# AI4Science-WestlakeU/RealPDEBench

Measured on AMD Instinct MI355X. Metric: train-step samples/sec (+ autoregressive rollout fields/sec in 'rollout'), FNO cylinder 128^2, higher is better.
Workload: dtype f32 storage / split-bf16x3 MFMA contractions (six bf16 products per fp32 product, fp32 accumulate), fp32-grade

## Files before the change

### include/rpb.h

```cpp
#ifndef RPB_H
#define RPB_H
#ifdef __cplusplus
extern "C" {
#endif

#define RPB_OK 0
#define RPB_ERR_ARG (-1)
#define RPB_ERR_LAUNCH (-2)
#define RPB_ERR_UNSUPPORTED (-3)

#define RPB_ABI_VERSION 3
const char* rpb_last_error(void);
int rpb_abi_version(void);
int rpb_bf16_const_planes(void);

int rpb_lift_pad_fwd(const float* x, const float* gt, const float* gh, const float* gw, const float* fc0_w,
                     const float* fc0_b, float* out, int B, int T, int H, int W, int Cin, int C, int Tp, int Hp, int Wp,
                     void* stream);
int rpb_lift_bwd_rows(void);
int rpb_lift_bwd(const float* g_out, const float* x, const float* gt, const float* gh, const float* gw, float* part,
                 int B, int T, int H, int W, int Cin, int C, int Tp, int Hp, int Wp, void* stream);

int rpb_axis_gemm(const float* in, float* out, const float* Mt, int G, int K, int O, int N, long in_g_stride,
                  long in_k_stride, long out_g_stride, long out_o_stride, int k_valid, int accumulate,
// ... 167 lines not shown
int rpb_col_reduce(const float* x, int ldx, float* part, int F, long n, int C, int mode, void* stream);

int rpb_feat_mix(const float* Phi, const float* w0, const float* b0, float* Xh, int B, int M2, int NB, int Cin, int C, void* stream);
int rpb_feat_mix_wgrad_rows(void);
int rpb_feat_mix_wgrad(const float* G, const float* Phi, float* part, int B, int M2, int NB, int Cin, int C, void* stream);
int rpb_small_gemm(const float* A, const float* Bm, float* out, int M, int N, int K, int a_rs, int a_cs, int b_rs, int b_cs,
                   int ldo, int accumulate, void* stream);
int rpb_lift_feat(const float* x, const float* gt, const float* gh, const float* gw, float* out, int B, int T, int H, int W,
                  int Cin, int Tp, int Hp, int Wp, int FW, void* stream);
int rpb_cell_mix_feat(const float* phi, const float* Wcomp, const float* bias, const float* z2, const float* GWt, float* out,
                      float* stats_part, long ncell, int FW, int K2, int Wp, const float* oxf_mean, const float* oxf_invstd,
                      const float* oxf_gamma, const float* oxf_beta, int oxf_gelu, void* stream);
int rpb_bn_bwd_row_feat(const float* s, const float* gy, const float* phi, float* gs, const float* mean, const float* invstd,
                        const float* gamma, const float* beta, const float* sums, double count, int gelu, const float* GWt,
                        float* Y1, float* part, int G, int Wp, int C, int K2, int FW, void* stream);

int rpb_bn_bwd_row_c128_supported(int Wp, int K2);
int rpb_bn_bwd_row_c128(const float* s, const float* gy, float* gs, const float* mean, const float* invstd, const float* gamma,
                        const float* beta, const float* sums, double count, int gelu, const float* GWt, float* Y1, float* part,
                        int G, int Wp, int K2, void* stream);

int rpb_proj_bwd_fused_supported(int C, int DO, int W, int Wp);
long rpb_proj_dgrad_slots(int B, int Tp, int Hp);
int rpb_proj_dgrad(const float* s, const float* w1, const float* gu, float* g, float* stats_part, int B, int DO, int T, int H, int W,
                   int Tp, int Hp, int Wp, const float* xf_mean, const float* xf_invstd, const float* xf_gamma, const float* xf_beta,
                   int xf_gelu, void* stream);

int rpb_head_bwd_supported(int C, int DO, int W, int Wp, int xf_gelu, int act);
long rpb_head_bwd_slots(int B, int T, int H);
int rpb_head_bwd_row(int DO);
// ... 140 lines not shown
```

### realpdebench_amd/_lib.py

```python
import ctypes
import os

_HERE = os.path.dirname(os.path.abspath(__file__))
ABI_VERSION = 3
LIB_PATH = os.environ.get("RPB_LIB_PATH") or os.path.join(_HERE, "csrc", "librpb_hip.so")

_P, _I, _L, _F, _D = ctypes.c_void_p, ctypes.c_int, ctypes.c_long, ctypes.c_float, ctypes.c_double
_T = {"p": _P, "i": _I, "l": _L, "f": _F, "d": _D}

SIGNATURES = {
    "rpb_last_error": (ctypes.c_char_p, ""),
    "rpb_abi_version": (_I, ""),
    "rpb_bf16_const_planes": (_I, ""),
    "rpb_lift_pad_fwd": (_I, "ppppppp" + "iiiiiiiii" + "p"),
    "rpb_lift_pad_fwd_bf16": (_I, "ppppppp" + "iiiiiiiii" + "p"),
    "rpb_axis_gemm_bf16in": (_I, "ppp" + "iiii" + "llll" + "i" + "p"),
    "rpb_cell_mix_bf16": (_I, "pppppp" + "l" + "iii" + "ppppi" + "i" + "p"),
    "rpb_axis_gemm_bf16out": (_I, "ppp" + "iiii" + "llll" + "i" + "p"),
    "rpb_proj_fwd_bf16": (_I, "pppppp" + "l" + "ii" + "iiiiii" + "i" + "p"),
    "rpb_spectrum_bin": (_I, "ppiip"),
    "rpb_feat_mix": (_I, "pppp" + "iiiii" + "p"),
    "rpb_feat_mix_wgrad_rows": (_I, ""),
    "rpb_feat_mix_wgrad": (_I, "ppp" + "iiiii" + "p"),
    "rpb_small_gemm": (_I, "ppp" + "iiiiiiiii" + "p"),
    "rpb_lift_feat": (_I, "ppppp" + "iiiiiiiii" + "p"),
    "rpb_cell_mix_feat": (_I, "ppppppp" + "l" + "iii" + "ppppi" + "p"),
    "rpb_bn_bwd_row_feat": (_I, "ppppppppp" + "d" + "i" + "ppp" + "iiiii" + "p"),
    "rpb_proj_bwd_fused_supported": (_I, "iiii"),
    "rpb_proj_dgrad_slots": (_L, "iii"),
    "rpb_proj_dgrad": (_I, "ppppp" + "ii" + "iiiiii" + "ppppi" + "p"),
    "rpb_stream_probe": (_I, "pppp" + "l" + "ii" + "p"),
    "rpb_mfma_probe": (_I, "pp" + "ii" + "p" + "p"),
    "rpb_head_bwd_supported": (_I, "iiiiii"),
    "rpb_head_bwd_slots": (_L, "iii"),
    "rpb_head_bwd_row": (_I, "i"),
    "rpb_head_bwd": (_I, "ppppppp" + "ii" + "iiiiii" + "pppp" + "p"),
    "rpb_head_bwd_finalize": (_I, "pppp" + "i" + "ppppp" + "p"),
    "rpb_head_fwd_bwd": (_I, "pppppp" + "f" + "ppp" + "ii" + "iiiiii" + "pppp" + "p"),
# ... 225 lines not shown
```

### realpdebench_amd/csrc/rpb_bwd_row.hip

```cpp
#include "rpb_common.h"
#include "rpb_bwr.h"
#include <stdlib.h>

template <int N>
struct RowVec;
template <>
struct RowVec<1> {
    typedef float T;
    typedef unsigned U;
};
template <>
struct RowVec<2> {
    typedef f32x2 T;
    typedef unsigned U __attribute__((ext_vector_type(2)));
};

template <int NT>
__device__ __forceinline__ typename RowVec<NT>::T row_load(rsrc_t r, int voff, int soff) {
    if constexpr (NT == 1) return __builtin_bit_cast(float, __builtin_amdgcn_raw_buffer_load_b32(r, voff, soff, RPB_STREAM_AUX));
    else return __builtin_bit_cast(f32x2, __builtin_amdgcn_raw_buffer_load_b64(r, voff, soff, RPB_STREAM_AUX));
}
template <int NT>
__device__ __forceinline__ void row_store(typename RowVec<NT>::T v, rsrc_t r, int voff, int soff) {
    if constexpr (NT == 1) __builtin_amdgcn_raw_buffer_store_b32(__builtin_bit_cast(unsigned, v), r, voff, soff, RPB_STREAM_AUX);
// ... 18 lines not shown
    const float* mean;
    const float* invstd;
    const float* gamma;
    const float* beta;
    const float* sums;
    float inv_count;
    int gelu;
    XForm xf;
    const float* GWt;
    float* Y1;
    float* part;
    int G, Wp, K2;
    int feat_w;
};

template <int C, bool FEAT = false>
__global__ __launch_bounds__(512) void bwd_row_kernel(BwdRowArgs a) {
    constexpr int NT = C / 32;
    typedef typename RowVec<NT>::T vec;
    extern __shared__ float Ml[];
    const int Wp = a.Wp, K2 = a.K2;
    const int nchunk = (Wp + 7) / 8;
    const int Kp = nchunk * 8;
    for (int idx = threadIdx.x; idx < Kp * 32; idx += blockDim.x) {
        const int k = idx >> 5, o = idx & 31;
        Ml[idx] = (k < Wp && o < K2) ? a.GWt[k * K2 + o] : 0.f;
    }
    __syncthreads();

    const int waves = blockDim.x >> 6;
    const int wave = __builtin_amdgcn_readfirstlane(threadIdx.x >> 6);
    const int lane = threadIdx.x & 63;
    const int col = lane & 31, half = lane >> 5;
    const long slot = (long)blockIdx.x * waves + wave;
    const long nslots = (long)gridDim.x * waves;
    const bool gelu = a.gelu != 0;
    const bool has_xf = !FEAT && a.xf.mean != nullptr;
    const int FW = a.feat_w;

    float mu[NT], is[NT], ga[NT], be[NT], m1[NT], m2[NT];
    XParam xp[NT];
#pragma unroll
    for (int t = 0; t < NT; ++t) {
        const int ch = col * NT + t;
        mu[t] = a.mean[ch];
        is[t] = a.invstd[ch];
        ga[t] = a.gamma[ch];
        be[t] = a.beta[ch];
        m1[t] = a.sums[ch] * a.inv_count;
        m2[t] = a.sums[C + ch] * a.inv_count;
        if (has_xf) xp[t] = xf_load(a.xf, ch);
    }
    f32x16 dW[NT][NT];
    float bsum[NT];
#pragma unroll
    for (int o = 0; o < NT; ++o) {
        bsum[o] = 0.f;
#pragma unroll
        for (int i = 0; i < NT; ++i) dW[o][i] = zero16();
    }

    const int voff = (half * C + col * NT) * 4;
    const unsigned row_bytes = (unsigned)Wp * C * 4;
    vec sa[4], ya[4], xa[4], sb[4], yb[4], xb[4];

    for (long g_ = slot; g_ < a.G; g_ += nslots) {
        const long g = (long)__builtin_amdgcn_readfirstlane((int)g_);
        const long off = g * (long)Wp * C;
        const rsrc_t rs = make_rsrc(a.s + off, row_bytes);
        const rsrc_t ry = make_rsrc(a.gy + off, row_bytes);
        const rsrc_t rx = FEAT ? make_rsrc(a.x + g * (long)Wp * FW, (unsigned)Wp * FW * 4u) : make_rsrc(a.x + off, row_bytes);
        const rsrc_t ro = make_rsrc(a.gs ? a.gs + off : a.s, a.gs ? row_bytes : 0u);
        f32x16 accw[NT];
#pragma unroll
        for (int t = 0; t < NT; ++t) accw[t] = zero16();

        auto load_chunk = [&](int c, vec (&sv)[4], vec (&yv)[4], vec (&xv)[4]) {
            const int vo = voff + c * 8 * C * 4;
#pragma unroll
            for (int j = 0; j < 4; ++j) {
                sv[j] = row_load<NT>(rs, vo + 2 * j * C * 4, 0);
                yv[j] = row_load<NT>(ry, vo + 2 * j * C * 4, 0);
                if (FEAT) {
                    const int fo = col < FW ? ((c * 8 + 2 * j + half) * FW + col) * 4 : 0x7ffffff0;
                    rset<NT>(xv[j], 0, buf_load_f32(rx, fo, 0));
                } else {
                    xv[j] = row_load<NT>(rx, vo + 2 * j * C * 4, 0);
                }
            }
        };
        auto compute_chunk = [&](int c, const vec (&sv)[4], const vec (&yv)[4], const vec (&xv)[4]) {
            const int vo = voff + c * 8 * C * 4;
            const float* mp = Ml + (c * 8 + half) * 32 + col;
#pragma unroll
            for (int j = 0; j < 4; ++j) {
                const bool valid = c * 8 + 2 * j + half < Wp;
                float gsv[NT], xt[NT];
                vec gout;
                if constexpr (NT == 2) {
                    const f32x2 isv = f32x2{is[0], is[1]}, gav = f32x2{ga[0], ga[1]};
                    const f32x2 sh = (sv[j] - f32x2{mu[0], mu[1]}) * isv;
                    f32x2 gz = yv[j];
                    if (gelu) gz = gz * gelu_grad2(pk_fma(sh, gav, f32x2{be[0], be[1]}));
                    f32x2 v = (gav * isv) * ((gz - f32x2{m1[0], m1[1]}) - sh * f32x2{m2[0], m2[1]});
                    v = valid ? v : pk2(0.f);
                    gout = v;
                    gsv[0] = v[0];
                    gsv[1] = v[1];
                    if (FEAT) {
                        xt[0] = xv[j][0];
                        xt[1] = 0.f;
                    } else {
                        f32x2 xx = xv[j];
                        if (has_xf) {
// ... 5 lines not shown
                        xt[1] = xx[1];
                    }
                } else {
#pragma unroll
                for (int t = 0; t < NT; ++t) {
                    const float sh = (rget<NT>(sv[j], t) - mu[t]) * is[t];
                    const float gyv = rget<NT>(yv[j], t);
                    const float gz = gelu ? gyv * gelu_grad_f(sh * ga[t] + be[t]) : gyv;
                    const float v = ga[t] * is[t] * (gz - m1[t] - sh * m2[t]);
                    gsv[t] = valid ? v : 0.f;
                    rset<NT>(gout, t, gsv[t]);
                    const float xv0 = (FEAT && t > 0) ? 0.f : rget<NT>(xv[j], t);
                    xt[t] = has_xf ? xf_apply(xv0, xp[t], a.xf.gelu != 0) : xv0;
                }
                }
                row_store<NT>(gout, ro, vo + 2 * j * C * 4, 0);
                const float aw = mp[2 * j * 32];
#pragma unroll
                for (int t = 0; t < NT; ++t) accw[t] = mfma32(aw, gsv[t], accw[t]);
#pragma unroll
                for (int o = 0; o < NT; ++o) {
                    bsum[o] += gsv[o];
#pragma unroll
                    for (int i = 0; i < (FEAT ? 1 : NT); ++i) dW[o][i] = mfma32(gsv[o], xt[i], dW[o][i]);
                }
            }
        };
        load_chunk(0, sa, ya, xa);
        for (int c = 0; c < nchunk; c += 2) {
            if (c + 1 < nchunk) load_chunk(c + 1, sb, yb, xb);
            compute_chunk(c, sa, ya, xa);
            if (c + 2 < nchunk) load_chunk(c + 2, sa, ya, xa);
            if (c + 1 < nchunk) compute_chunk(c + 1, sb, yb, xb);
        }
        float* yp = a.Y1 + g * (long)K2 * C + col * NT;
#pragma unroll
        for (int r = 0; r < 16; ++r) {
            const int o = mfma_row(lane, r);
            if (o < K2) {
                vec v;
#pragma unroll
                for (int t = 0; t < NT; ++t) rset<NT>(v, t, accw[t][r]);
                *reinterpret_cast<vec*>(yp + (long)o * C) = v;
            }
        }
    }
    float* part = a.part + slot * ((long)C * C + C);
#pragma unroll
    for (int o = 0; o < NT; ++o) {
#pragma unroll
        for (int i = 0; i < (FEAT ? 1 : NT); ++i)
#pragma unroll
            for (int r = 0; r < 16; ++r)
                part[(long)(mfma_row(lane, r) * NT + o) * C + (FEAT ? col : col * NT + i)] = dW[o][i][r];
        const float b = bsum[o] + __shfl_xor(bsum[o], 32, 64);
        if (half == 0) part[(long)C * C + col * NT + o] = b;
    }
}

extern "C" long rpb_bn_bwd_row_slots(int G) {
    const long slots = (long)rpb_num_cus() * 8;
    const long need = ((long)G + 7) / 8 * 8;
    return slots < need ? slots : need;
}

extern "C" int rpb_bn_bwd_row(const float* s, const float* gy, const float* x, float* gs, const float* mean,
                              const float* invstd, const float* gamma, const float* beta, const float* sums,
                              double count, int gelu, const float* xf_mean, const float* xf_invstd,
                              const float* xf_gamma, const float* xf_beta, int xf_gelu, const float* GWt, float* Y1,
                              float* part, int G, int Wp, int C, int K2, void* stream) {
    RPB_REQUIRE(s && gy && gs && mean && invstd && gamma && beta && sums && GWt && Y1 && part,
// ... 35 lines not shown
        BwrArgs b;
        b.s = s; b.gy = gy; b.x = nullptr; b.gs = gs;
        b.mean = mean + 64 * h; b.invstd = invstd + 64 * h; b.gamma = gamma + 64 * h; b.beta = beta + 64 * h; b.sums = sums + 64 * h;
        b.inv_count = (float)(1.0 / count); b.gelu = gelu; b.xf = XForm{nullptr, nullptr, nullptr, nullptr, 0};
        b.GW = GWt; b.Y1 = Y1; b.part = part + h * rows * (64 * 64 + 64); b.G = G; b.Wp = Wp; b.K2 = K2; b.CS = 128; b.coff = 64 * h;
        const int rc = rpb_bwr_launch(b, rows, (hipStream_t)stream);
        if (rc != RPB_OK) return rc;
    }
    return RPB_OK;
}

extern "C" int rpb_bn_bwd_row_feat(const float* s, const float* gy, const float* phi, float* gs, const float* mean,
                                   const float* invstd, const float* gamma, const float* beta, const float* sums, double count,
                                   int gelu, const float* GWt, float* Y1, float* part, int G, int Wp, int C, int K2, int FW,
                                   void* stream) {
    RPB_REQUIRE(s && gy && phi && mean && invstd && gamma && beta && sums && GWt && Y1 && part, "bn_bwd_row_feat: null pointer");
    RPB_REQUIRE(C == 64 && (FW == 8 || FW == 32), "bn_bwd_row_feat: C=%d FW=%d unsupported", C, FW);
    RPB_REQUIRE(G > 0 && Wp > 0 && K2 > 0 && K2 <= 32 && count > 0, "bn_bwd_row_feat: bad sizes G=%d Wp=%d K2=%d", G, Wp, K2);
    BwdRowArgs a;
    a.s = s; a.gy = gy; a.x = phi; a.gs = gs; a.mean = mean; a.invstd = invstd; a.gamma = gamma; a.beta = beta;
    a.sums = sums; a.inv_count = (float)(1.0 / count); a.gelu = gelu;
    a.xf = XForm{nullptr, nullptr, nullptr, nullptr, 0};
    a.GWt = GWt; a.Y1 = Y1; a.part = part; a.G = G; a.Wp = Wp; a.K2 = K2; a.feat_w = FW;
    const int grid = (int)(rpb_bn_bwd_row_slots(G) / 8);
    const size_t lds = (size_t)((Wp + 7) / 8 * 8) * 32 * 4;
    hipLaunchKernelGGL((bwd_row_kernel<64, true>), dim3(grid), dim3(512), lds, (hipStream_t)stream, a);
    RPB_CHECK_LAUNCH("bn_bwd_row_feat");
}
```

### realpdebench_amd/dft.py

```python
import math

import numpy as np
import torch


def kept_modes(n, m, two_sided):
    ks = list(range(m))
    if two_sided:
        if 2 * m > n:
            raise ValueError(f"modes {m} overlap on an axis of length {n} (2*modes must be <= padded size)")
        ks += list(range(n - m, n))
    elif m > n // 2 + 1:
        raise ValueError(f"modes {m} exceed the rfft length {n // 2 + 1}")
    return ks


def _fwd_complex(n, ks):
    k = np.asarray(ks, dtype=np.float64)[:, None]
    p = np.arange(n, dtype=np.float64)[None, :]
    th = 2.0 * math.pi * ((k * p) % n) / n
    c, s = np.cos(th), np.sin(th)
    M = np.zeros((2, len(ks), n, 2))
    M[0, :, :, 0] = c
    M[0, :, :, 1] = s
# ... 41 lines not shown
        self.kw = kept_modes(Wp, m3, False)
        self.KT, self.KH, self.KW = len(self.kt), len(self.kh), len(self.kw)
        self.M = self.KT * self.KH * self.KW
        mats = {
            "FW": _fwd_real(Wp, self.kw),
            "FH": _fwd_complex(Hp, self.kh),
            "FT": _fwd_complex(Tp, self.kt),
            "GT": _inv_complex(Tp, self.kt),
            "GH": _inv_complex(Hp, self.kh),
            "GW": _inv_real(Wp, self.kw, float(Tp) * Hp * Wp),
        }
        for name, m in mats.items():
            t = torch.from_numpy(np.ascontiguousarray(m)).to(torch.float32)
            setattr(self, name, t.to(device).contiguous())
            setattr(self, name + "t", t.t().contiguous().to(device))


def ref_weights_to_mode_major(w1, w2, w3, w4):
    top = torch.cat([w1, w3], dim=3)
    bot = torch.cat([w2, w4], dim=3)
    full = torch.cat([top, bot], dim=2)
    full = full.permute(2, 3, 4, 0, 1).contiguous()
    return torch.view_as_real(full).reshape(-1, full.shape[3], full.shape[4], 2).contiguous()


def mode_major_to_ref_weights(wm, modes):
    m1, m2, m3 = modes
    Ci, Co = wm.shape[1], wm.shape[2]
    full = torch.view_as_complex(wm.reshape(2 * m1, 2 * m2, m3, Ci, Co, 2).contiguous())
    full = full.permute(3, 4, 0, 1, 2)
# ... 6 lines not shown
```

### realpdebench_amd/model/fno.py

```python
import math
import os
from collections import OrderedDict

import numpy as np
import torch
import torch.nn as nn

from .. import ops
from ..dft import SpectralPlan, mode_major_to_ref_weights, ref_weights_to_mode_major
from .model import Model

HID = 128
BN_EPS = 1e-5
BN_MOMENTUM = 0.1
_ALIGN = 64


class _Workspace:

    def __init__(self, model, B, training, device):
        d = ops.Dims(B, *model.shape_in[:3], model.dim_in, model.width, model.padding)
        self.d, self.training = d, training
        self.bf16 = (not training) and model.storage == "bf16"
        self.arith = model.arith if (not training and not self.bf16) else "f32"
# ... 44 lines not shown
            phi[..., c0 + 1] = grids[1].view(1, H_, 1)
            phi[..., c0 + 2] = grids[2].view(1, 1, W_)
            phi[..., c0 + 3] = 1.0
            self.phi = phi
            n1 = 2 * plan.KW * self.NB
            self.fy1 = torch.empty(T_ * H_ * n1, **f)
            self.fy2 = torch.empty(T_ * 2 * plan.KH * plan.KW * self.NB, **f)
            self.PhiH = torch.empty(2 * plan.M * self.NB, **f)
            if training:
                self.fm_rows = ops.feat_mix_wgrad_rows()
                self.fm_part = torch.empty(self.fm_rows * C * (Cin + 4), **f)
                self.fm_sum = torch.empty(C * (Cin + 4), **f)
                self.mgf = torch.empty(C * (Cin + 3) + C, **f)
                self.mgf2 = torch.empty(C * C, **f)
                self.dconv = torch.empty(C * (Cin + 4), **f)
        if training:
            self.G = [torch.empty(d.ncell, C, **f) for _ in range(2)]
            self.proj_gu = (C == 64 and type(model)._lift_fwd is FNO3d._lift_fwd
                            and ops.proj_bwd_fused_supported(C, model.dim_out, d.W, d.Wp))
            self.head_fused = (C == 64 and type(model)._lift_fwd is FNO3d._lift_fwd and
                               ops.head_bwd_supported(C, model.dim_out, d.W, d.Wp, False, model.proj_act))
            self.gu = None if self.head_fused else torch.empty(d.ncrop, HID, **f)
            if self.proj_gu:
                self.pd_slots = ops.proj_dgrad_slots(d)
            if self.head_fused:
                self.hb_slots, self.hb_row = ops.head_bwd_slots(d), ops.head_bwd_row(model.dim_out)
                self.hb_part = torch.empty(self.hb_slots * self.hb_row, **f)
                self.hb_tot = torch.empty(self.hb_row, **f)
                self.hb_loss_part = torch.empty(self.hb_slots, **f)
                self.head_loss_fused = model.dim_out <= 2
# ... 310 lines not shown
        world = self.dp.world_size if (self.dp is not None and training) else 1
        a_in, xf = ws.A0, None
        y1_ready = False
        for l in range(L):
            s = ws.S[l] if training else ws.S[l % 2]
            xh = ws.Xh[l] if training else ws.Xh[0]
            if dpw is not None:
                dpw.params_ready(dpw.layer_bucket(l))
            if l == 0 and ws.feat0:
                self._feature_spectrum(x, ws, plan)
                ops.feat_mix(ws.PhiH, P("fc0.weight"), P("fc0.bias"), xh, d.B, 2 * plan.M, ws.NB, self.dim_in, C)
            elif y1_ready:
                self._spectral_forward_stages(a_in, ws, xh, (None, plan.FHt, plan.FTt), first_layer=False, y1=ws.Y1f)
            else:
                self._spectral_forward_stages(a_in, ws, xh, (plan.FWt, plan.FHt, plan.FTt), first_layer=(l == 0), xf=xf)
            ops.mode_contract_fwd(xh, P(f"spec.{l}"), ws.Yh, d.B, plan.M, C)
            self._spectral_inverse_stages(ws.Yh, ws, (plan.GTt, plan.GHt))
            if training:
                if l == 0 and ws.featfull:
                    ops.cell_mix_feat(ws.phic, ws.wcomp, P("convs.0.bias"), ws.Y1, plan.GWt, s, ws.stat_part, d.ncell, ws.FW,
                                      2 * plan.KW, d.Wp)
                else:
                    ops.cell_mix(a_in, P(f"convs.{l}.weight"), P(f"convs.{l}.bias"), ws.Y1, plan.GWt, s, ws.stat_part,
                                 d.ncell, C, C, 2 * plan.KW, d.Wp, xf=xf)
                ops.reduce_partials(ws.stat_part, ws.stat_rows, 2 * C, out_f64=ws.sums64)
                if world > 1 or (self.dp is not None and training and getattr(self.dp, "sync_stats_always", False)):
                    self.dp.all_reduce_sum(ws.sums64)
                ops.bn_finalize(ws.sums64, float(d.ncell) * world, BN_EPS, BN_MOMENTUM, ws.mean[l], ws.invstd[l],
                                self.bn_running_mean[l], self.bn_running_var[l], C)
                self.bn_num_batches_tracked[l] += 1
                a_in, xf = s, self._layer_xf(ws, l, True)
            else:
                ops.bn_eval_prep(self.bn_running_var[l], BN_EPS, ws.invstd[l], C)
                y1_ready = False
                if ws.fuse_w and l < L - 1 and (l > 0 or ws.featfull or ws.bf16):
                    feat = l == 0 and ws.featfull
                    ops.cell_mix_eval_dft(ws.phic if feat else a_in, ws.wcomp if feat else P(f"convs.{l}.weight"), P(f"convs.{l}.bias"),
                                          ws.Z2, plan.GWt, s, d.ncell, 2 * plan.KW, d.Wp, self._layer_xf(ws, l, False), plan.FWt,
                                          2 * plan.KW, ws.Y1f, feat_w=ws.FW if feat else 0, arith=ws.arith, spec_e=ops.spec_exp(d))
                    y1_ready = True
                elif l == 0 and ws.featfull:
                    ops.cell_mix_feat(ws.phic, ws.wcomp, P("convs.0.bias"), ws.Z2, plan.GWt, s, None, d.ncell, ws.FW,
                                      2 * plan.KW, d.Wp, oxf=self._layer_xf(ws, l, False))
# ... 62 lines not shown
                ops.cell_mix(ws.gu, P("fc1.weight"), None, None, None, g, ws.bn_part, d.ncell, HID, C, 0, 1, transpose_w=True,
                             gather=True, crop6=d.crop6, bnb=(ws.S[L - 1],) + self._layer_xf(ws, L - 1, True))
                ops.reduce_partials(ws.bn_part, ws.bnb_rows_gather, 2 * C, out_f32=ws.bn_sums)
        gz_ok = ws.fused_bwd and ops.cell_mix_writes_gz(d.ncell, C, C, 2 * plan.KW, d.Wp, True)
        g_is_gz = False
        for l in range(L - 1, -1, -1):
            gelu = l < L - 1 and not g_is_gz
            gam, bet = P(f"bns.{l}.weight"), P(f"bns.{l}.bias")
            GP(f"bns.{l}.bias").copy_(ws.bn_sums[:C])
            GP(f"bns.{l}.weight").copy_(ws.bn_sums[C:])
            if world > 1 or (self.dp is not None and getattr(self.dp, "sync_stats_always", False)):
                self.dp.all_reduce_sum(ws.bn_sums)
            a_in = ws.A0 if l == 0 else ws.S[l - 1]
            xf_in = None if l == 0 else self._layer_xf(ws, l - 1, True)
            feat_l0 = l == 0 and ws.featfull
            if feat_l0:
                ops.bn_bwd_row_feat(ws.S[l], g, ws.phic, None if ws.feat0 else g, ws.mean[l], ws.invstd[l], gam, bet, ws.bn_sums,
                                    float(d.ncell) * world, gelu, plan.GW, ws.Y1, ws.wg_part, d.B * d.Tp * d.Hp, d.Wp, C,
                                    2 * plan.KW, ws.FW)
            elif ws.fused_bwd:
                wg_later = ws.wg_in_cmx and l > 0
                ops.bn_bwd_row(ws.S[l], g, None if wg_later else a_in, g, ws.mean[l], ws.invstd[l], gam, bet, ws.bn_sums,
                               float(d.ncell) * world, gelu, xf_in, plan.GW, ws.Y1, ws.wg_part, d.B * d.Tp * d.Hp,
                               d.Wp, C, 2 * plan.KW)
            elif ws.row128:
                ops.bn_bwd_row_c128(ws.S[l], g, g, ws.mean[l], ws.invstd[l], gam, bet, ws.bn_sums, float(d.ncell) * world, gelu,
                                    plan.GW, ws.Y1, ws.row128_part, d.B * d.Tp * d.Hp, d.Wp, 2 * plan.KW)
                ops.cell_wgrad(g, a_in, ws.wg_part, d.ncell, C, C, xf=xf_in)
            else:
                ops.bn_bwd_apply(ws.S[l], g, ws.mean[l], ws.invstd[l], gam, bet, ws.bn_sums, float(d.ncell) * world,
                                 g, d.ncell, C, gelu)
                ops.cell_wgrad(g, a_in, ws.wg_part, d.ncell, C, C, xf=xf_in)
            partc = ws.wg_part[:ws.wg_rows_c * (C * C + C)].view(ws.wg_rows_c, C * C + C)
            if feat_l0:
                self._reduce_cols(partc, 0, C * C, ws.mgf2)
                ops.small_gemm(ws.mgf2, ws.w0ext, GP("convs.0.weight"), C, C, ws.FW, C, 1, 1, ws.FW, C)
            elif not (ws.fused_bwd and ws.wg_in_cmx and l > 0):
                self._reduce_cols(partc, 0, C * C, GP(f"convs.{l}.weight"))
            self._reduce_cols(partc, C * C, C, GP(f"convs.{l}.bias"))
            self._spectral_forward_stages(g, ws, ws.Yh, (None if (ws.fused_bwd or ws.row128) else plan.GW, plan.GH, plan.GT),
                                          first_layer=False)
            ops.mode_contract_wgrad(ws.Xh[l], ws.Yh, GP(f"spec.{l}"), d.B, plan.M, C)
            if self.dp is not None:
                self.dp.bucket_ready(gflat, hold_small_of=l if (ws.fused_bwd and ws.wg_in_cmx and l > 0) else None)
            gxh = ws.Xh[l]
            ops.mode_contract_dgrad(ws.Yh, P(f"spec.{l}"), gxh, d.B, plan.M, C)
            if l == 0 and ws.feat0:
                Cin, F = self.dim_in, self.dim_in + 3
                ops.feat_mix_wgrad(gxh, ws.PhiH, ws.fm_part, d.B, 2 * plan.M, ws.NB, Cin, C)
                ops.reduce_partials(ws.fm_part, ws.fm_rows, C * (F + 1), out_f32=ws.fm_sum)
                tot = ws.fm_sum.view(C, F + 1)
                GP("fc0.weight").copy_(tot[:, :F])
                GP("fc0.bias").copy_(tot[:, F])
                wc = P("convs.0.weight")
                if ws.featfull:
                    ops.small_gemm(wc, ws.mgf2, ws.dconv, C, F + 1, C, 1, C, C, 1, F + 1)
# ... 111 lines not shown
```

### realpdebench_amd/ops.py

```python
import os
import threading

import torch

from . import _lib

F32 = torch.float32


def _stream():
    return torch.cuda.current_stream().cuda_stream


class Sub:

    def __init__(self, t, offset):
        self.t, self.offset = t, int(offset)


def _p(t, dtype=F32):
    if t is None:
        return None
    if isinstance(t, Sub):
        return _p(t.t, dtype) + 4 * t.offset
# ... 861 lines not shown

def feat_mix(Phi, w0, b0, Xh, B, M2, NB, Cin, C):
    _lib.call("rpb_feat_mix", _p(Phi), _p(w0), _p(b0), _p(Xh), B, M2, NB, Cin, C, _stream(), label="feat_mix",
              nbytes=4 * B * M2 * C)


def feat_mix_wgrad_rows():
    return _lib.query("rpb_feat_mix_wgrad_rows")


def feat_mix_wgrad(G, Phi, part, B, M2, NB, Cin, C):
    _lib.call("rpb_feat_mix_wgrad", _p(G), _p(Phi), _p(part), B, M2, NB, Cin, C, _stream(), label="feat_mix_wgrad",
              nbytes=4 * B * M2 * C)


def small_gemm(A, Bm, out, M, N, K, a_rs, a_cs, b_rs, b_cs, ldo, accumulate=False):
    _lib.call("rpb_small_gemm", _p(A), _p(Bm), _p(out), M, N, K, a_rs, a_cs, b_rs, b_cs, ldo, int(accumulate), _stream(),
              label="small_gemm")


def lift_feat(x, grids, out, d, FW):
    _lib.call("rpb_lift_feat", _p(x), _p(grids[0]), _p(grids[1]), _p(grids[2]), _p(out), d.B, d.T, d.H, d.W, d.Cin, d.Tp, d.Hp,
              d.Wp, FW, _stream(), label="lift_feat", nbytes=4 * (d.ncrop * d.Cin + d.ncell * FW))


def cell_mix_feat(phi, Wcomp, bias, z2, GW, out, stats_part, ncell, FW, K2, Wp, oxf=None):
    _lib.call("rpb_cell_mix_feat", _p(phi), _p(Wcomp), _p(bias), _p(z2), _p(GW), _p(out), _p(stats_part), ncell, FW, K2, Wp,
              *_xf(oxf), _stream(), label=f"cell_mix[feat{FW}->CO64,spec=1,stats={'oxf' if oxf is not None else int(stats_part is not None)}]",
              nbytes=4 * (ncell * (FW + 64) + (ncell // Wp) * K2 * 64), flops=2 * ncell * 64 * (K2 + FW))


def bn_bwd_row_feat(s, gy, phi, gs, mean, invstd, gamma, beta, sums, count, gelu, GWt, Y1, part, G, Wp, C, K2, FW):
    _lib.call("rpb_bn_bwd_row_feat", _p(s), _p(gy), _p(phi), _p(gs), _p(mean), _p(invstd), _p(gamma), _p(beta), _p(sums),
              float(count), int(gelu), _p(GWt), _p(Y1), _p(part), G, Wp, C, K2, FW, _stream(),
              label=f"bn_bwd_row[C{C},feat{FW}{'' if gs is not None else ',nogs'}]",
              nbytes=4 * ((3 if gs is not None else 2) * G * Wp * C + G * Wp * FW + G * K2 * C),
              flops=2 * G * Wp * C * (FW + K2))


def dpot_patch_tokens(u, gx, gy, gt, P, B, T, H, W, Cd, Cm, ps):
    _lib.call("rpb_dpot_patch_tokens", _p(u), _p(gx), _p(gy), _p(gt), _p(P), B, T, H, W, Cd, Cm, ps, _stream(),
              label="dpot_patch_tokens", nbytes=4 * (u.numel() + P.numel()))


def dpot_patch_tokens_bwd(gP, gu, B, T, H, W, Cd, Cm, ps):
    _lib.call("rpb_dpot_patch_tokens_bwd", _p(gP), _p(gu), B, T, H, W, Cd, Cm, ps, _stream(), label="dpot_patch_tokens_bwd",
              nbytes=4 * (gu.numel() + gP.numel()))
# ... 58 lines not shown
```

Baseline: 906.5.

## Apply layer-0 BatchNorm backward correction in spectral space instead of per cell

For layer 0 in training, the per-cell BN backward (which reads the saved activation S and writes gs) becomes a raw pass that only accumulates weight moments from the incoming gradient. The BN mean and variance correction terms are then applied afterwards to the much smaller spectral buffer and to the moment matrix, using new kernels l0_spectrum_fix and l0_moment_fix. This removes a full-grid read of S and some per-cell arithmetic. In exchange it adds an extra Yh0 buffer, two small kernels, a partial reduction, fp64 sums and extra algebraic complexity.

```diff
diff --git a/include/rpb.h b/include/rpb.h
--- a/include/rpb.h
+++ b/include/rpb.h
@@ -205,6 +205,14 @@
 int rpb_bn_bwd_row_feat(const float* s, const float* gy, const float* phi, float* gs, const float* mean, const float* invstd,
                         const float* gamma, const float* beta, const float* sums, double count, int gelu, const float* GWt,
                         float* Y1, float* part, int G, int Wp, int C, int K2, int FW, void* stream);
+int rpb_l0_spectrum_fix(float* Gh, const float* X0, const float* Y0, const float* Wc, const float* bias, const float* mean,
+                        const float* invstd, const float* gamma, const float* sums, double count, const float* adjw,
+                        const int* partner, const float* PhiH, float* qpart, int B, int M, int KW, int C, int NB, int Cin,
+                        void* stream);
+int rpb_l0_spectrum_fix_rows(void);
+int rpb_l0_moment_fix(float* mgf, float* dbias, const float* q, const float* wcomp, const float* bias, const float* mean,
+                      const float* invstd, const float* gamma, const float* sums, double count, const double* ssum, double ncell,
+                      int C, int FW, int Cin, void* stream);
 
 int rpb_bn_bwd_row_c128_supported(int Wp, int K2);
 int rpb_bn_bwd_row_c128(const float* s, const float* gy, float* gs, const float* mean, const float* invstd, const float* gamma,
diff --git a/realpdebench_amd/_lib.py b/realpdebench_amd/_lib.py
--- a/realpdebench_amd/_lib.py
+++ b/realpdebench_amd/_lib.py
@@ -22,6 +22,9 @@
     "rpb_feat_mix": (_I, "pppp" + "iiiii" + "p"),
     "rpb_feat_mix_wgrad_rows": (_I, ""),
     "rpb_feat_mix_wgrad": (_I, "ppp" + "iiiii" + "p"),
+    "rpb_l0_spectrum_fix_rows": (_I, ""),
+    "rpb_l0_spectrum_fix": (_I, "ppppppppp" + "d" + "pppp" + "iiiiii" + "p"),
+    "rpb_l0_moment_fix": (_I, "ppppppppp" + "d" + "p" + "d" + "iii" + "p"),
     "rpb_small_gemm": (_I, "ppp" + "iiiiiiiii" + "p"),
     "rpb_lift_feat": (_I, "ppppp" + "iiiiiiiii" + "p"),
     "rpb_cell_mix_feat": (_I, "ppppppp" + "l" + "iii" + "ppppi" + "p"),
diff --git a/realpdebench_amd/csrc/rpb_bwd_row.hip b/realpdebench_amd/csrc/rpb_bwd_row.hip
--- a/realpdebench_amd/csrc/rpb_bwd_row.hip
+++ b/realpdebench_amd/csrc/rpb_bwd_row.hip
@@ -56,8 +56,10 @@
     int feat_w;
 };
 
-template <int C, bool FEAT = false>
+template <int C, bool FEAT = false, int RAW = 0>
 __global__ __launch_bounds__(512) void bwd_row_kernel(BwdRowArgs a) {
+    static_assert(!RAW || (FEAT && C == 64), "the raw mode exists for the layer-0 instance only");
+    constexpr bool VAL = RAW == 2;
     constexpr int NT = C / 32;
     typedef typename RowVec<NT>::T vec;
     extern __shared__ float Ml[];
@@ -84,6 +86,7 @@
     XParam xp[NT];
 #pragma unroll
     for (int t = 0; t < NT; ++t) {
+        if constexpr (RAW) break;
         const int ch = col * NT + t;
         mu[t] = a.mean[ch];
         is[t] = a.invstd[ch];
@@ -101,6 +104,12 @@
 #pragma unroll
         for (int i = 0; i < NT; ++i) dW[o][i] = zero16();
     }
+    f32x16 dG = zero16();
+    float mr[NT][8], gm[2] = {0.f, 0.f};
+#pragma unroll
+    for (int t = 0; t < NT; ++t)
+#pragma unroll
+        for (int f = 0; f < 8; ++f) mr[t][f] = 0.f;
 
     const int voff = (half * C + col * NT) * 4;
     const unsigned row_bytes = (unsigned)Wp * C * 4;
@@ -109,7 +118,7 @@
     for (long g_ = slot; g_ < a.G; g_ += nslots) {
         const long g = (long)__builtin_amdgcn_readfirstlane((int)g_);
         const long off = g * (long)Wp * C;
-        const rsrc_t rs = make_rsrc(a.s + off, row_bytes);
+        const rsrc_t rs = RAW ? make_rsrc(a.gy, 0u) : make_rsrc(a.s + off, row_bytes);
         const rsrc_t ry = make_rsrc(a.gy + off, row_bytes);
         const rsrc_t rx = FEAT ? make_rsrc(a.x + g * (long)Wp * FW, (unsigned)Wp * FW * 4u) : make_rsrc(a.x + off, row_bytes);
         const rsrc_t ro = make_rsrc(a.gs ? a.gs + off : a.s, a.gs ? row_bytes : 0u);
@@ -121,7 +130,7 @@
             const int vo = voff + c * 8 * C * 4;
 #pragma unroll
             for (int j = 0; j < 4; ++j) {
-                sv[j] = row_load<NT>(rs, vo + 2 * j * C * 4, 0);
+                if constexpr (!RAW) sv[j] = row_load<NT>(rs, vo + 2 * j * C * 4, 0);
                 yv[j] = row_load<NT>(ry, vo + 2 * j * C * 4, 0);
                 if (FEAT) {
                     const int fo = col < FW ? ((c * 8 + 2 * j + half) * FW + col) * 4 : 0x7ffffff0;
@@ -139,7 +148,27 @@
                 const bool valid = c * 8 + 2 * j + half < Wp;
                 float gsv[NT], xt[NT];
                 vec gout;
-                if constexpr (NT == 2) {
+                if constexpr (RAW) {
+#pragma unroll
+                    for (int t = 0; t < NT; ++t) {
+                        gsv[t] = rget<NT>(yv[j], t);
+                        xt[t] = t == 0 ? rget<NT>(xv[j], 0) : 0.f;
+                    }
+                    if constexpr (VAL) {
+                        const int hb = lane & 32;
+#pragma unroll
+                        for (int f = 0; f < 8; ++f) {
+                            const float ph = __shfl(xt[0], hb + f, 64);
+#pragma unroll
+                            for (int t = 0; t < NT; ++t) mr[t][f] = fmaf(gsv[t], ph, mr[t][f]);
+                        }
+                        const float pa = __shfl(xt[0], hb + (col & 7), 64);
+                        gm[0] = fmaf(pa, __shfl(xt[0], hb + (col >> 3), 64), gm[0]);
+                        gm[1] = fmaf(pa, __shfl(xt[0], hb + 4 + (col >> 3), 64), gm[1]);
+                    } else {
+                        dG = mfma32(xt[0], xt[0], dG);
+                    }
+                } else if constexpr (NT == 2) {
                     const f32x2 isv = f32x2{is[0], is[1]}, gav = f32x2{ga[0], ga[1]};
                     const f32x2 sh = (sv[j] - f32x2{mu[0], mu[1]}) * isv;
                     f32x2 gz = yv[j];
@@ -175,13 +204,14 @@
                     xt[t] = has_xf ? xf_apply(xv0, xp[t], a.xf.gelu != 0) : xv0;
                 }
                 }
-                row_store<NT>(gout, ro, vo + 2 * j * C * 4, 0);
+                if constexpr (!RAW) row_store<NT>(gout, ro, vo + 2 * j * C * 4, 0);
                 const float aw = mp[2 * j * 32];
 #pragma unroll
                 for (int t = 0; t < NT; ++t) accw[t] = mfma32(aw, gsv[t], accw[t]);
 #pragma unroll
                 for (int o = 0; o < NT; ++o) {
                     bsum[o] += gsv[o];
+                    if constexpr (VAL) continue;
 #pragma unroll
                     for (int i = 0; i < (FEAT ? 1 : NT); ++i) dW[o][i] = mfma32(gsv[o], xt[i], dW[o][i]);
                 }
@@ -212,10 +242,28 @@
 #pragma unroll
         for (int i = 0; i < (FEAT ? 1 : NT); ++i)
 #pragma unroll
-            for (int r = 0; r < 16; ++r)
-                part[(long)(mfma_row(lane, r) * NT + o) * C + (FEAT ? col : col * NT + i)] = dW[o][i][r];
+            for (int r = 0; r < 16; ++r) {
+                if constexpr (VAL) {
+                    if (r < 8) {
+                        const float m = mr[o][r] + __shfl_xor(mr[o][r], 32, 64);
+                        if (half == 0) part[(long)(col * NT + o) * C + r] = m;
+                    }
+                } else {
+                    part[(long)(mfma_row(lane, r) * NT + o) * C + (FEAT ? col : col * NT + i)] = dW[o][i][r];
+                }
+            }
         const float b = bsum[o] + __shfl_xor(bsum[o], 32, 64);
         if (half == 0) part[(long)C * C + col * NT + o] = b;
+    }
+    if constexpr (VAL) {
+#pragma unroll
+        for (int k = 0; k < 2; ++k) {
+            const float v = gm[k] + __shfl_xor(gm[k], 32, 64);
+            if (half == 0) part[(long)(4 * k + (col >> 3)) * C + 32 + (col & 7)] = v;
+        }
+    } else if constexpr (RAW != 0) {
+#pragma unroll
+        for (int r = 0; r < 16; ++r) part[(long)mfma_row(lane, r) * C + 32 + col] = dG[r];
     }
 }
 
@@ -281,16 +329,21 @@
                                    const float* invstd, const float* gamma, const float* beta, const float* sums, double count,
                                    int gelu, const float* GWt, float* Y1, float* part, int G, int Wp, int C, int K2, int FW,
                                    void* stream) {
-    RPB_REQUIRE(s && gy && phi && mean && invstd && gamma && beta && sums && GWt && Y1 && part, "bn_bwd_row_feat: null pointer");
+    const bool raw = s == nullptr;
+    RPB_REQUIRE(gy && phi && GWt && Y1 && part && (raw ? !gs && !gelu : mean && invstd && gamma && beta && sums && count > 0),
+                "bn_bwd_row_feat: null pointer");
     RPB_REQUIRE(C == 64 && (FW == 8 || FW == 32), "bn_bwd_row_feat: C=%d FW=%d unsupported", C, FW);
-    RPB_REQUIRE(G > 0 && Wp > 0 && K2 > 0 && K2 <= 32 && count > 0, "bn_bwd_row_feat: bad sizes G=%d Wp=%d K2=%d", G, Wp, K2);
+    RPB_REQUIRE(G > 0 && Wp > 0 && K2 > 0 && K2 <= 32, "bn_bwd_row_feat: bad sizes G=%d Wp=%d K2=%d", G, Wp, K2);
+    RPB_REQUIRE((long)Wp * C * 4 < (1L << 31), "bn_bwd_row_feat: row too long");
     BwdRowArgs a;
     a.s = s; a.gy = gy; a.x = phi; a.gs = gs; a.mean = mean; a.invstd = invstd; a.gamma = gamma; a.beta = beta;
-    a.sums = sums; a.inv_count = (float)(1.0 / count); a.gelu = gelu;
+    a.sums = sums; a.inv_count = raw ? 0.f : (float)(1.0 / count); a.gelu = gelu;
     a.xf = XForm{nullptr, nullptr, nullptr, nullptr, 0};
     a.GWt = GWt; a.Y1 = Y1; a.part = part; a.G = G; a.Wp = Wp; a.K2 = K2; a.feat_w = FW;
     const int grid = (int)(rpb_bn_bwd_row_slots(G) / 8);
     const size_t lds = (size_t)((Wp + 7) / 8 * 8) * 32 * 4;
-    hipLaunchKernelGGL((bwd_row_kernel<64, true>), dim3(grid), dim3(512), lds, (hipStream_t)stream, a);
+    if (raw && FW == 8) hipLaunchKernelGGL((bwd_row_kernel<64, true, 2>), dim3(grid), dim3(512), lds, (hipStream_t)stream, a);
+    else if (raw) hipLaunchKernelGGL((bwd_row_kernel<64, true, 1>), dim3(grid), dim3(512), lds, (hipStream_t)stream, a);
+    else hipLaunchKernelGGL((bwd_row_kernel<64, true>), dim3(grid), dim3(512), lds, (hipStream_t)stream, a);
     RPB_CHECK_LAUNCH("bn_bwd_row_feat");
 }
diff --git a/realpdebench_amd/csrc/rpb_l0spec.hip b/realpdebench_amd/csrc/rpb_l0spec.hip
--- /dev/null
+++ b/realpdebench_amd/csrc/rpb_l0spec.hip
@@ -0,0 +1,113 @@
+#include "rpb_common.h"
+
+#define L0_FMAX 24
+__global__ __launch_bounds__(256) void l0_spectrum_fix_kernel(float* __restrict__ Gh, const float* __restrict__ X0,
+                                                              const float* __restrict__ Y0, const float* __restrict__ Wc,
+                                                              const float* __restrict__ bias, const float* __restrict__ mean,
+                                                              const float* __restrict__ invstd, const float* __restrict__ gamma,
+                                                              const float* __restrict__ sums, float inv_count,
+                                                              const float* __restrict__ adjw, const int* __restrict__ partner,
+                                                              const float* __restrict__ PhiH, float* __restrict__ qpart, int B, int M,
+                                                              int KW, int NB, int Cin) {
+    __shared__ float red[4][64 * L0_FMAX];
+    const int lane = threadIdx.x & 63, wv = threadIdx.x >> 6;
+    const int wave = blockIdx.x * 4 + wv, nwaves = gridDim.x * 4;
+    const int F1 = Cin + 4;
+    const int rows = B * 2 * M;
+    float w[64];
+#pragma unroll
+    for (int j = 0; j < 64; j += 4) {
+        const f32x4 v = *reinterpret_cast<const f32x4*>(Wc + lane * 64 + j);
+#pragma unroll
+        for (int k = 0; k < 4; ++k) w[j + k] = v[k];
+    }
+    const float is = invstd[lane], gis = gamma[lane] * is;
+    const float m1 = sums[lane] * inv_count, m2is = sums[64 + lane] * inv_count * is;
+    const float dc = gis * (m1 + m2is * (bias[lane] - mean[lane]));
+    float q[L0_FMAX];
+#pragma unroll
+    for (int f = 0; f < L0_FMAX; ++f) q[f] = 0.f;
+    for (int row_ = wave; row_ < rows; row_ += nwaves) {
+        const int row = __builtin_amdgcn_readfirstlane(row_);
+        const int b = row / (2 * M), rm = row - b * 2 * M;
+        const int ri = rm >= M, m = rm - ri * M;
+        const int kw = m % KW, kth = m / KW;
+        const long at = (long)row * 64 + lane;
+        const float x = X0[at];
+        float acc[4] = {0.f, 0.f, 0.f, 0.f};
+#pragma unroll
+        for (int j = 0; j < 64; ++j)
+            acc[j & 3] = fmaf(w[j], __builtin_bit_cast(float, __builtin_amdgcn_readlane(__builtin_bit_cast(int, x), j)), acc[j & 3]);
+        const float mix = (acc[0] + acc[1]) + (acc[2] + acc[3]);
+        const float y0 = Y0[at], D = adjw[kw];
+        float y = y0;
+        if (adjw[2 * KW + kw] != 0.f) {
+            const int p = partner[kth];
+            if (p >= 0) {
+                const float yp = Y0[((long)(row - m) + (long)p * KW + kw) * 64 + lane];
+                y += ri ? -yp : yp;
+            }
+        }
+        float out = gis * (Gh[at] - m2is * (D * mix + adjw[KW + kw] * y));
+        if (m == 0 && ri == 0) out -= dc;
+        Gh[at] = out;
+        const float dy = D * y0;
+        const float* ph = PhiH + (long)rm * NB;
+#pragma unroll
+        for (int f = 0; f < L0_FMAX; ++f)
+            if (f < F1) q[f] = fmaf(dy, f < Cin ? ph[b * Cin + f] : ph[B * Cin + (f - Cin)], q[f]);
+    }
+#pragma unroll
+    for (int f = 0; f < L0_FMAX; ++f)
+        if (f < F1) red[wv][lane * F1 + f] = q[f];
+    __syncthreads();
+    for (int idx = threadIdx.x; idx < 64 * F1; idx += blockDim.x)
+        qpart[(long)blockIdx.x * 64 * F1 + idx] = (red[0][idx] + red[1][idx]) + (red[2][idx] + red[3][idx]);
+}
+
+extern "C" int rpb_l0_spectrum_fix_rows(void) { return rpb_num_cus() * 8; }
+
+extern "C" int rpb_l0_spectrum_fix(float* Gh, const float* X0, const float* Y0, const float* Wc, const float* bias, const float* mean,
+                                   const float* invstd, const float* gamma, const float* sums, double count, const float* adjw,
+                                   const int* partner, const float* PhiH, float* qpart, int B, int M, int KW, int C, int NB, int Cin,
+                                   void* stream) {
+    RPB_REQUIRE(Gh && X0 && Y0 && Wc && bias && mean && invstd && gamma && sums && adjw && partner && PhiH && qpart,
+                "l0_spectrum_fix: null pointer");
+    RPB_REQUIRE(C == 64 && B > 0 && M > 0 && KW > 0 && M % KW == 0 && count > 0, "l0_spectrum_fix: bad sizes B=%d M=%d KW=%d C=%d", B, M, KW, C);
+    RPB_REQUIRE(Cin > 0 && Cin + 4 <= L0_FMAX && NB >= B * Cin + 4, "l0_spectrum_fix: bad field sizes Cin=%d NB=%d", Cin, NB);
+    RPB_REQUIRE((long)B * 2 * M < (1L << 24), "l0_spectrum_fix: too many rows");
+    hipLaunchKernelGGL(l0_spectrum_fix_kernel, dim3(rpb_l0_spectrum_fix_rows()), dim3(256), 0, (hipStream_t)stream, Gh, X0, Y0, Wc, bias,
+                       mean, invstd, gamma, sums, (float)(1.0 / count), adjw, partner, PhiH, qpart, B, M, KW, NB, Cin);
+    RPB_CHECK_LAUNCH("l0_spectrum_fix");
+}
+
+__global__ __launch_bounds__(256) void l0_moment_fix_kernel(float* mgf, float* dbias, const float* __restrict__ q,
+                                                            const float* __restrict__ wcomp, const float* __restrict__ bias,
+                                                            const float* __restrict__ mean, const float* __restrict__ invstd,
+                                                            const float* __restrict__ gamma, const float* __restrict__ sums,
+                                                            double inv_count, const double* __restrict__ ssum, double ncell, int FW,
+                                                            int F1) {
+    const int C = 64;
+    for (int idx = threadIdx.x; idx < C * FW; idx += blockDim.x) {
+        const int c = idx / FW, f = idx - c * FW;
+        const double is = invstd[c], gis = (double)gamma[c] * is, mu = mean[c];
+        const double m1 = sums[c] * inv_count, m2is = sums[C + c] * inv_count * is;
+        const double sphi = mgf[(F1 - 1) * C + 32 + f];
+        double wg = 0.0;
+        for (int j = 0; j < FW; ++j) wg += (double)wcomp[c * FW + j] * (double)mgf[j * C + 32 + f];
+        const double qv = f < F1 ? (double)q[c * F1 + f] : 0.0;
+        const double out = gis * ((double)mgf[c * C + f] - m1 * sphi - m2is * (wg + ((double)bias[c] - mu) * sphi + qv));
+        if (f == 0) dbias[c] = (float)(gis * ((double)dbias[c] - ncell * m1 - m2is * (ssum[c] - ncell * mu)));
+        mgf[c * C + f] = (float)out;
+    }
+}
+
+extern "C" int rpb_l0_moment_fix(float* mgf, float* dbias, const float* q, const float* wcomp, const float* bias, const float* mean,
+                                 const float* invstd, const float* gamma, const float* sums, double count, const double* ssum,
+                                 double ncell, int C, int FW, int Cin, void* stream) {
+    RPB_REQUIRE(mgf && dbias && q && wcomp && bias && mean && invstd && gamma && sums && ssum, "l0_moment_fix: null pointer");
+    RPB_REQUIRE(C == 64 && (FW == 8 || FW == 32) && Cin > 0 && Cin + 4 <= FW && count > 0 && ncell > 0, "l0_moment_fix: bad sizes C=%d FW=%d Cin=%d", C, FW, Cin);
+    hipLaunchKernelGGL(l0_moment_fix_kernel, dim3(1), dim3(256), 0, (hipStream_t)stream, mgf, dbias, q, wcomp, bias, mean, invstd, gamma, sums,
+                       1.0 / count, ssum, ncell, FW, Cin + 4);
+    RPB_CHECK_LAUNCH("l0_moment_fix");
+}
diff --git a/realpdebench_amd/dft.py b/realpdebench_amd/dft.py
--- a/realpdebench_amd/dft.py
+++ b/realpdebench_amd/dft.py
@@ -79,6 +79,33 @@
             t = torch.from_numpy(np.ascontiguousarray(m)).to(torch.float32)
             setattr(self, name, t.to(device).contiguous())
             setattr(self, name + "t", t.t().contiguous().to(device))
+        D, R, selfc = adjoint_weights(Tp, Hp, Wp, self.kw)
+        self.adjD64, self.adjR64, self.self_conj = D, R, selfc
+        self.partner_host = conj_partner(Tp, Hp, self.kt, self.kh)
+        adjw = np.stack([D, R, selfc.astype(np.float64)])
+        self.adjw = torch.from_numpy(adjw).to(torch.float32).to(device).contiguous()
+        self.partner = torch.from_numpy(self.partner_host).to(torch.int32).to(device).contiguous()
+
+
+def adjoint_weights(Tp, Hp, Wp, kw):
+    n = float(Tp) * Hp * Wp
+    k = np.asarray(kw)
+    selfc = (k == 0) | ((Wp % 2 == 0) & (k == Wp // 2))
+    D = np.where(selfc, 1.0, 2.0) / n
+    R = np.where(selfc, 0.5, 2.0) / n
+    return D, R, selfc
+
+
+def conj_partner(Tp, Hp, kt, kh):
+    pt = {f: i for i, f in enumerate(kt)}
+    ph = {f: i for i, f in enumerate(kh)}
+    out = np.full(len(kt) * len(kh), -1, dtype=np.int64)
+    for it, ft in enumerate(kt):
+        for ih, fh in enumerate(kh):
+            jt, jh = pt.get((Tp - ft) % Tp), ph.get((Hp - fh) % Hp)
+            if jt is not None and jh is not None:
+                out[it * len(kh) + ih] = jt * len(kh) + jh
+    return out
 
 
 def ref_weights_to_mode_major(w1, w2, w3, w4):
diff --git a/realpdebench_amd/model/fno.py b/realpdebench_amd/model/fno.py
--- a/realpdebench_amd/model/fno.py
+++ b/realpdebench_amd/model/fno.py
@@ -82,6 +82,15 @@
                 self.mgf = torch.empty(C * (Cin + 3) + C, **f)
                 self.mgf2 = torch.empty(C * C, **f)
                 self.dconv = torch.empty(C * (Cin + 4), **f)
+        self.l0_spectral = (training and self.featfull and self.feat0 and C == 64
+                            and os.environ.get("RPB_L0_SPECTRAL_BN", "1") != "0")
+        if self.l0_spectral:
+            self.Yh0 = torch.empty(B * 2 * plan.M * C, **f)
+            self.sums64_l0 = torch.empty(2 * C, device=device, dtype=torch.float64)
+            self.s0_local = torch.empty(C, device=device, dtype=torch.float64)
+            self.l0_q = torch.empty(C * (model.dim_in + 4), **f)
+            self.l0_qrows = ops.l0_spectrum_fix_rows()
+            self.l0_qpart = torch.empty(self.l0_qrows * C * (model.dim_in + 4), **f)
         if training:
             self.G = [torch.empty(d.ncell, C, **f) for _ in range(2)]
             self.proj_gu = (C == 64 and type(model)._lift_fwd is FNO3d._lift_fwd
@@ -422,8 +431,11 @@
                 self._spectral_forward_stages(a_in, ws, xh, (None, plan.FHt, plan.FTt), first_layer=False, y1=ws.Y1f)
             else:
                 self._spectral_forward_stages(a_in, ws, xh, (plan.FWt, plan.FHt, plan.FTt), first_layer=(l == 0), xf=xf)
-            ops.mode_contract_fwd(xh, P(f"spec.{l}"), ws.Yh, d.B, plan.M, C)
-            self._spectral_inverse_stages(ws.Yh, ws, (plan.GTt, plan.GHt))
+            l0_spec = l == 0 and training and ws.l0_spectral
+            yh = ws.Yh0 if l0_spec else ws.Yh
+            sums64 = ws.sums64_l0 if l0_spec else ws.sums64
+            ops.mode_contract_fwd(xh, P(f"spec.{l}"), yh, d.B, plan.M, C)
+            self._spectral_inverse_stages(yh, ws, (plan.GTt, plan.GHt))
             if training:
                 if l == 0 and ws.featfull:
                     ops.cell_mix_feat(ws.phic, ws.wcomp, P("convs.0.bias"), ws.Y1, plan.GWt, s, ws.stat_part, d.ncell, ws.FW,
@@ -431,10 +443,15 @@
                 else:
                     ops.cell_mix(a_in, P(f"convs.{l}.weight"), P(f"convs.{l}.bias"), ws.Y1, plan.GWt, s, ws.stat_part,
                                  d.ncell, C, C, 2 * plan.KW, d.Wp, xf=xf)
-                ops.reduce_partials(ws.stat_part, ws.stat_rows, 2 * C, out_f64=ws.sums64)
+                ops.reduce_partials(ws.stat_part, ws.stat_rows, 2 * C, out_f64=sums64)
                 if world > 1 or (self.dp is not None and training and getattr(self.dp, "sync_stats_always", False)):
-                    self.dp.all_reduce_sum(ws.sums64)
-                ops.bn_finalize(ws.sums64, float(d.ncell) * world, BN_EPS, BN_MOMENTUM, ws.mean[l], ws.invstd[l],
+                    if l0_spec:
+                        ws.s0_local.copy_(sums64[:C])
+                    self.dp.all_reduce_sum(sums64)
+                    ws.s0_sum = ws.s0_local
+                elif l0_spec:
+                    ws.s0_sum = sums64
+                ops.bn_finalize(sums64, float(d.ncell) * world, BN_EPS, BN_MOMENTUM, ws.mean[l], ws.invstd[l],
                                 self.bn_running_mean[l], self.bn_running_var[l], C)
                 self.bn_num_batches_tracked[l] += 1
                 a_in, xf = s, self._layer_xf(ws, l, True)
@@ -527,7 +544,11 @@
             a_in = ws.A0 if l == 0 else ws.S[l - 1]
             xf_in = None if l == 0 else self._layer_xf(ws, l - 1, True)
             feat_l0 = l == 0 and ws.featfull
-            if feat_l0:
+            l0_spec = feat_l0 and ws.l0_spectral and not gelu
+            if l0_spec:
+                ops.bn_bwd_row_feat(None, g, ws.phic, None, None, None, None, None, None, 1.0, False, plan.GW, ws.Y1, ws.wg_part,
+                                    d.B * d.Tp * d.Hp, d.Wp, C, 2 * plan.KW, ws.FW)
+            elif feat_l0:
                 ops.bn_bwd_row_feat(ws.S[l], g, ws.phic, None if ws.feat0 else g, ws.mean[l], ws.invstd[l], gam, bet, ws.bn_sums,
                                     float(d.ncell) * world, gelu, plan.GW, ws.Y1, ws.wg_part, d.B * d.Tp * d.Hp, d.Wp, C,
                                     2 * plan.KW, ws.FW)
@@ -547,12 +568,21 @@
             partc = ws.wg_part[:ws.wg_rows_c * (C * C + C)].view(ws.wg_rows_c, C * C + C)
             if feat_l0:
                 self._reduce_cols(partc, 0, C * C, ws.mgf2)
-                ops.small_gemm(ws.mgf2, ws.w0ext, GP("convs.0.weight"), C, C, ws.FW, C, 1, 1, ws.FW, C)
+                if not l0_spec:
+                    ops.small_gemm(ws.mgf2, ws.w0ext, GP("convs.0.weight"), C, C, ws.FW, C, 1, 1, ws.FW, C)
             elif not (ws.fused_bwd and ws.wg_in_cmx and l > 0):
                 self._reduce_cols(partc, 0, C * C, GP(f"convs.{l}.weight"))
             self._reduce_cols(partc, C * C, C, GP(f"convs.{l}.bias"))
             self._spectral_forward_stages(g, ws, ws.Yh, (None if (ws.fused_bwd or ws.row128) else plan.GW, plan.GH, plan.GT),
                                           first_layer=False)
+            if l0_spec:
+                bn0 = (P("convs.0.bias"), ws.mean[0], ws.invstd[0], gam, ws.bn_sums, float(d.ncell) * world)
+                ops.l0_spectrum_fix(ws.Yh, ws.Xh[0], ws.Yh0, P("convs.0.weight"), *bn0, plan.adjw, plan.partner, ws.PhiH, ws.l0_qpart,
+                                    d.B, plan.M, plan.KW, C, ws.NB, self.dim_in)
+                ops.reduce_partials(ws.l0_qpart, ws.l0_qrows, C * (self.dim_in + 4), out_f32=ws.l0_q)
+                ops.l0_moment_fix(ws.mgf2, GP("convs.0.bias"), ws.l0_q, ws.wcomp, *bn0, ws.s0_sum, float(d.ncell), C, ws.FW,
+                                  self.dim_in)
+                ops.small_gemm(ws.mgf2, ws.w0ext, GP("convs.0.weight"), C, C, ws.FW, C, 1, 1, ws.FW, C)
             ops.mode_contract_wgrad(ws.Xh[l], ws.Yh, GP(f"spec.{l}"), d.B, plan.M, C)
             if self.dp is not None:
                 self.dp.bucket_ready(gflat, hold_small_of=l if (ws.fused_bwd and ws.wg_in_cmx and l > 0) else None)
diff --git a/realpdebench_amd/ops.py b/realpdebench_amd/ops.py
--- a/realpdebench_amd/ops.py
+++ b/realpdebench_amd/ops.py
@@ -899,6 +899,21 @@
               nbytes=4 * B * M2 * C)
 
 
+def l0_spectrum_fix_rows():
+    return _lib.query("rpb_l0_spectrum_fix_rows")
+
+
+def l0_spectrum_fix(Gh, X0, Y0, Wc, bias, mean, invstd, gamma, sums, count, adjw, partner, PhiH, qpart, B, M, KW, C, NB, Cin):
+    _lib.call("rpb_l0_spectrum_fix", _p(Gh), _p(X0), _p(Y0), _p(Wc), _p(bias), _p(mean), _p(invstd), _p(gamma), _p(sums), float(count),
+              _p(adjw), _p(partner, torch.int32), _p(PhiH), _p(qpart), B, M, KW, C, NB, Cin, _stream(), label="l0_spectrum_fix",
+              nbytes=4 * (4 * B * 2 * M * C + 2 * M * NB), flops=2 * B * 2 * M * C * (C + Cin + 4))
+
+
+def l0_moment_fix(mgf, dbias, q, wcomp, bias, mean, invstd, gamma, sums, count, ssum, ncell, C, FW, Cin):
+    _lib.call("rpb_l0_moment_fix", _p(mgf), _p(dbias), _p(q), _p(wcomp), _p(bias), _p(mean), _p(invstd), _p(gamma), _p(sums),
+              float(count), _p(ssum, torch.float64), float(ncell), C, FW, Cin, _stream(), label="l0_moment_fix")
+
+
 def small_gemm(A, Bm, out, M, N, K, a_rs, a_cs, b_rs, b_cs, ldo, accumulate=False):
     _lib.call("rpb_small_gemm", _p(A), _p(Bm), _p(out), M, N, K, a_rs, a_cs, b_rs, b_cs, ldo, int(accumulate), _stream(),
               label="small_gemm")
@@ -916,6 +931,11 @@
 
 
 def bn_bwd_row_feat(s, gy, phi, gs, mean, invstd, gamma, beta, sums, count, gelu, GWt, Y1, part, G, Wp, C, K2, FW):
+    if s is None:
+        _lib.call("rpb_bn_bwd_row_feat", None, _p(gy), _p(phi), None, None, None, None, None, None, 1.0, 0, _p(GWt), _p(Y1), _p(part),
+                  G, Wp, C, K2, FW, _stream(), label=f"bn_bwd_row[C{C},feat{FW},raw]",
+                  nbytes=4 * (G * Wp * C + G * Wp * FW + G * K2 * C), flops=2 * G * Wp * (C * (FW + K2) + 32 * 32))
+        return
     _lib.call("rpb_bn_bwd_row_feat", _p(s), _p(gy), _p(phi), _p(gs), _p(mean), _p(invstd), _p(gamma), _p(beta), _p(sums),
               float(count), int(gelu), _p(GWt), _p(Y1), _p(part), G, Wp, C, K2, FW, _stream(),
               label=f"bn_bwd_row[C{C},feat{FW}{'' if gs is not None else ',nogs'}]",
```

Result: no change. 911.0, median of 6 (+0.5%).
